# weiyithu/PV-RAFT

Measured on NVIDIA H100. Metric: raft_sample_iters_per_sec, higher is better.
Workload: dtype f32

## Files before the change

pvraft_b200/csrc/corr_lookup.cu:

```cuda
#include <math.h>

#include "fixed_point.cuh"
#include "tma.cuh"

namespace pvraft {

constexpr int kLookupThreads = 640;
constexpr int kAccCells = 128;

__host__ __device__ constexpr size_t lookup_warp_bytes(int K) {
    return (((size_t)(K < 512 ? 512 : K) * 2 + (size_t)K * 4 + 256 + 128 + 2 * kAccCells * 4 + 16) + 127) & ~(size_t)127;
}

struct LookupParams {
    const void* corr_val;
    const void* corr_idx;
    const float4* tab;
    const float* coords;
    float* vox;
    float4* knn_sel;
    int32_t* knn_slot;
    double* moments;
    int8_t* dbg_cube;
    int B, N, K, levels;
    int M;
    int vox_ld;
    float r[4];
    float inv_r[4];
    float thr_c;
    int warps;
    int chunk;
};

template <bool POW2>
__device__ __forceinline__ float div_r(float d, float r, float inv_r) {
    return POW2 ? __fmul_rn(d, inv_r) : __fdiv_rn(d, r);
}

template <bool POW2>
__device__ __forceinline__ unsigned cell_code(float dx, float dy, float dz, float r, float inv_r) {
    const float qx = rintf(div_r<POW2>(dx, r, inv_r));
    const float qy = rintf(div_r<POW2>(dy, r, inv_r));
    const float qz = rintf(div_r<POW2>(dz, r, inv_r));
    const bool ok = fmaxf(fmaxf(fabsf(qx), fabsf(qy)), fabsf(qz)) <= 1.f;
    const int cell = (int)fmaf(qx, 9.f, fmaf(qy, 3.f, qz + 13.f));
    return ok ? (unsigned)cell : 0xFFu;
}

__device__ __forceinline__ void prefetch_row(const void* row, int bytes, int lane) {
    const char* r = reinterpret_cast<const char*>(row);
    if (bytes <= 2048) {
        if (lane * 64 < bytes) asm volatile("prefetch.global.L2 [%0];" ::"l"(r + lane * 64));
    } else {
        for (int o = lane * 64; o < bytes; o += 32 * 64) asm volatile("prefetch.global.L2 [%0];" ::"l"(r + o));
    }
}

template <bool HALF> struct StateT { using val = float; using idx = int32_t; };
template <> struct StateT<true> { using val = uint16_t; using idx = uint16_t; };
__device__ __forceinline__ float load_val(const float* p) { return __ldg(p); }
__device__ __forceinline__ float load_val(const uint16_t* p) { return __uint_as_float((unsigned)__ldg(p) << 16); }

__device__ __forceinline__ unsigned warp_scan_packed(unsigned w, int lane) {
#pragma unroll
    for (int o = 1; o < 32; o <<= 1) {
        const unsigned a = __shfl_up_sync(kFull, w, o);
        if (lane >= o) w += a;
    }
    return w;
}

__device__ __forceinline__ double moments_reduce_scatter(double (&v)[16], int lane) {
#pragma unroll
    for (int d = 16, h = 8; d >= 2; d >>= 1, h >>= 1) {
        const bool up = (lane & d) != 0;
#pragma unroll
        for (int i = 0; i < h; ++i) {
            const double send = up ? v[i] : v[i + h];
            const double keep = up ? v[i + h] : v[i];
            v[i] = keep + __shfl_xor_sync(kFull, send, d);
        }
    }
    return v[0] + __shfl_xor_sync(kFull, v[0], 1);
}

template <int KPL, bool POW2, bool SMEM_TAB, bool HALF, bool DET>
__global__ void __launch_bounds__(kLookupThreads, 1) k_corr_lookup(const LookupParams p) {
    using val_t = typename StateT<HALF>::val;
    using idx_t = typename StateT<HALF>::idx;
    const val_t* g_val = reinterpret_cast<const val_t*>(p.corr_val);
    const idx_t* g_idx = reinterpret_cast<const idx_t*>(p.corr_idx);
    constexpr int VEC = KPL >= 4 ? 4 : KPL;
    constexpr int NJ = KPL / VEC;
    constexpr int K = KPL * 32;
    constexpr unsigned NIB = (1u << VEC) - 1u;
    extern __shared__ __align__(128) unsigned char smem_raw[];
    const size_t tab_bytes = SMEM_TAB ? (((size_t)p.M * 16 + 127) & ~(size_t)127) : 0;
    const float4* s_tab = reinterpret_cast<const float4*>(smem_raw);
    const int w = warp_id();
    int lane;
    asm volatile("mov.u32 %0, %%laneid;" : "=r"(lane));
    unsigned char* wbase = smem_raw + tab_bytes + (size_t)w * lookup_warp_bytes(K);
    int* s_stage = reinterpret_cast<int*>(wbase);
    constexpr int VL = (K < 512 ? 512 : K) * 2;
    unsigned short* s_vlist = reinterpret_cast<unsigned short*>(wbase + K * 4);
    int* s_hist = reinterpret_cast<int*>(wbase + K * 4);
    int* s_slots = reinterpret_cast<int*>(wbase + K * 4 + VL + 256);
    float* s_acc = reinterpret_cast<float*>(wbase + K * 4 + VL + 384);
    int* s_cnt = reinterpret_cast<int*>(wbase + K * 4 + VL + 384 + kAccCells * 4);
    unsigned long long* s_bar = reinterpret_cast<unsigned long long*>(wbase + K * 4 + VL + 384 + 2 * kAccCells * 4);
    pdl_trigger();
    const bool active_warp = w < p.warps;
    __shared__ int s_next;
    __shared__ unsigned long long s_tabbar;
    double* s_rcp = reinterpret_cast<double*>(smem_raw + tab_bytes + (size_t)p.warps * lookup_warp_bytes(K));
    for (int i = threadIdx.x; i <= K; i += blockDim.x) s_rcp[i] = i > 0 ? 1.0 / (double)min(i, p.N) : 1.0;

    if (active_warp && lane == 0) mbar_init(s_bar, 1);
    if (threadIdx.x == 0) mbar_init(&s_tabbar, 1);
    fence_mbarrier_init();
    __syncthreads();

    const bool dyn = p.moments != nullptr && (int)gridDim.x >= p.B;
    const long long total = (long long)p.B * p.N;
    long long pt_begin, pt_end;
    if (dyn) {
        const int b = (int)((long long)blockIdx.x * p.B / gridDim.x);
        pt_begin = (long long)b * p.N;
        pt_end = pt_begin + p.N;
    } else {
        split_range(total, gridDim.x, blockIdx.x, pt_begin, pt_end);
    }
    const int L = p.levels;
    const int nvox = L * 27;
    const unsigned lt_mask = (1u << lane) - 1u;
    unsigned phase = 0, tab_phase = 0;
    bool waited = false;
    const int kChunk = p.chunk;
    const unsigned one = (unsigned)min(p.chunk, 1);

    long long seg = pt_begin;
    while (seg < pt_end) {
        const int b = (int)(seg / p.N);
        long long seg_end = (long long)(b + 1) * p.N;
        if (seg_end > pt_end) seg_end = pt_end;
        const float4* tab_g = p.tab + (size_t)b * p.M;
        int* counter = dyn ? reinterpret_cast<int*>(p.moments + (size_t)b * PVRAFT_MOMENTS + 15) : nullptr;
        if constexpr (DET)
            counter = dyn ? reinterpret_cast<int*>(reinterpret_cast<unsigned long long*>(p.moments) + ((size_t)b * PVRAFT_MOMENTS + 15) * kFxWords) : nullptr;
        auto claim_chunk = [&]() -> long long {
            int c = 0;
            if (lane == 0) c = atomicAdd(counter, kChunk);
            return seg + __shfl_sync(kFull, c, 0);
        };
        __syncthreads();
        if (SMEM_TAB && threadIdx.x == 0) {
            asm volatile("fence.proxy.async.shared::cta;" ::: "memory");
            const unsigned bytes = (unsigned)p.M * 16u;
            mbar_expect_tx(&s_tabbar, bytes);
            for (unsigned off = 0; off < bytes; off += 32768u)
                bulk_g2s(smem_raw + off, reinterpret_cast<const unsigned char*>(tab_g) + off, min(32768u, bytes - off), &s_tabbar);
        }
        if (threadIdx.x == 0) s_next = 2 * p.warps;
        if (!waited) { pdl_wait(); waited = true; }
        long long pt0 = seg + w, nxt0 = seg + w + p.warps;
        int left0 = 0;
        if (dyn && active_warp) { pt0 = claim_chunk(); nxt0 = pt0 + 1; left0 = kChunk - 2; }
        if (active_warp && pt0 < seg_end) {
            if (lane == 0) {
                mbar_expect_tx(s_bar, K * sizeof(idx_t));
                bulk_g2s(s_stage, g_idx + pt0 * K, K * sizeof(idx_t), s_bar);
            }
            prefetch_row(g_val + pt0 * K, K * sizeof(val_t), lane);
        }
        if (SMEM_TAB) { mbar_wait(&s_tabbar, tab_phase); tab_phase ^= 1u; }
        __syncthreads();
        double mom[14];
#pragma unroll
        for (int i = 0; i < 14; ++i) mom[i] = 0.0;
        Fx fmom{0ull, 0ull, 0u};

        if (active_warp) {
            int left = left0, done = 0;
            long long nxt = nxt0;
            for (long long pt = pt0; pt < seg_end; ++done) {
                const float cx = __ldg(p.coords + pt * 3 + 0);
                const float cy = __ldg(p.coords + pt * 3 + 1);
                const float cz = __ldg(p.coords + pt * 3 + 2);
                const val_t* rv = g_val + pt * K;
                const idx_t* ri = g_idx + pt * K;
                if (p.dbg_cube) {
                    for (int i = lane; i < K * L; i += 32) p.dbg_cube[pt * K * L + i] = (int8_t)-1;
                }
                *reinterpret_cast<float4*>(s_acc + lane * 4) = make_float4(0.f, 0.f, 0.f, 0.f);
                *reinterpret_cast<int4*>(s_cnt + lane * 4) = make_int4(0, 0, 0, 0);
                mbar_wait(s_bar, phase);
                phase ^= 1u;

                unsigned dist[KPL];
                unsigned valid_bits = 0;
                const float thr = p.thr_c;
#pragma unroll
                for (int j = 0; j < NJ; ++j) {
                    int ci[VEC];
                    if (VEC == 4 && HALF) {
                        const uint2 c = reinterpret_cast<const uint2*>(s_stage)[j * 32 + lane];
                        ci[0] = (int)(c.x & 0xFFFFu); ci[1 % VEC] = (int)(c.x >> 16); ci[2 % VEC] = (int)(c.y & 0xFFFFu); ci[3 % VEC] = (int)(c.y >> 16);
                    } else if (VEC == 4) {
                        const int4 c = reinterpret_cast<const int4*>(s_stage)[j * 32 + lane];
                        ci[0] = c.x; ci[1 % VEC] = c.y; ci[2 % VEC] = c.z; ci[3 % VEC] = c.w;
                    } else {
#pragma unroll
                        for (int s = 0; s < VEC; ++s) ci[s] = (int)reinterpret_cast<const idx_t*>(s_stage)[j * 32 * VEC + lane * VEC + s];
                    }
#pragma unroll
                    for (int s = 0; s < VEC; ++s) {
                        const float4 q = SMEM_TAB ? s_tab[ci[s]] : __ldg(tab_g + ci[s]);
                        const float dx = __fsub_rn(q.x, cx), dy = __fsub_rn(q.y, cy);
                        const float sx = __fmul_rn(dx, dx), sy = __fmul_rn(dy, dy);
                        const float dz = __fsub_rn(q.z, cz);
                        const float d2 = __fadd_rn(__fadd_rn(sx, sy), __fmul_rn(dz, dz));
                        dist[j * VEC + s] = __float_as_uint(d2);
                        const float amax = fmaxf(fmaxf(fabsf(dx), fabsf(dy)), fabsf(dz));
                        valid_bits |= (amax < thr ? 1u : 0u) << (j * VEC + s);
                    }
                }
                __syncwarp();
                if (nxt < seg_end) {
                    if (lane == 0) {
                        asm volatile("fence.proxy.async.shared::cta;" ::: "memory");
                        mbar_expect_tx(s_bar, K * sizeof(idx_t));
                        bulk_g2s(s_stage, g_idx + nxt * K, K * sizeof(idx_t), s_bar);
                    }
                    prefetch_row(g_val + nxt * K, K * sizeof(val_t), lane);
                }

                if (__any_sync(kFull, valid_bits != 0u)) {
                    int list_n = 0;
                    unsigned w0 = 0, w1 = 0;
#pragma unroll
                    for (int j = 0; j < NJ; ++j) {
                        const unsigned c = __popc((valid_bits >> (j * VEC)) & NIB);
                        if (j < 4) w0 |= c << (8 * j); else w1 |= c << (8 * (j - 4));
                    }
                    const unsigned i0 = warp_scan_packed(w0, lane);
                    const unsigned t0 = __shfl_sync(kFull, i0, 31);
                    unsigned i1 = 0, t1 = 0;
                    if (NJ > 4) { i1 = warp_scan_packed(w1, lane); t1 = __shfl_sync(kFull, i1, 31); }
                    const unsigned e0 = i0 - w0, e1 = i1 - w1;
#pragma unroll
                    for (int j = 0; j < NJ; ++j) {
                        const unsigned ex = j < 4 ? (e0 >> (8 * j)) & 0xFFu : (e1 >> (8 * (j - 4))) & 0xFFu;
                        const unsigned tt = j < 4 ? (t0 >> (8 * j)) & 0xFFu : (t1 >> (8 * (j - 4))) & 0xFFu;
                        unsigned nib = (valid_bits >> (j * VEC)) & NIB;
                        int pos = list_n + (int)ex;
                        while (nib) {
                            const int s = __ffs(nib) - 1;
                            nib &= nib - 1;
                            s_vlist[pos++] = (unsigned short)(j * 32 * VEC + lane * VEC + s);
                        }
                        list_n += (int)tt;
                    }
                    __syncwarp();
                    for (int c0 = 0; c0 < list_n; c0 += 32) {
                        const int n = min(32, list_n - c0);
                        unsigned code = 0xFFFFFFFFu;
                        float val = 0.f;
                        if (lane < n) {
                            const int slot = s_vlist[c0 + lane];
                            const int id = (int)__ldg(ri + slot);
                            val = load_val(rv + slot);
                            const float4 q = SMEM_TAB ? s_tab[id] : __ldg(tab_g + id);
                            const float dx = __fsub_rn(q.x, cx), dy = __fsub_rn(q.y, cy), dz = __fsub_rn(q.z, cz);
#pragma unroll
                            for (int l = 0; l < 4; ++l) {
                                if (l < L) {
                                    const unsigned c = cell_code<POW2>(dx, dy, dz, p.r[l], p.inv_r[l]);
                                    code = (code & ~(0xFFu << (8 * l))) | (c << (8 * l));
                                    if (p.dbg_cube) p.dbg_cube[(pt * K + slot) * L + l] = (int8_t)c;
                                }
                            }
                        }
#pragma unroll
                        for (int l = 0; l < 4; ++l) {
                            if (l < L) {
                                const unsigned c = (code >> (8 * l)) & 0xFFu;
                                const bool act = c != 0xFFu;
                                if (__any_sync(kFull, act)) {
                                    const unsigned m = __match_any_sync(kFull, c);
                                    const unsigned rank = __popc(m & lt_mask), gsize = __popc(m);
                                    const unsigned maxg = __reduce_max_sync(kFull, act ? gsize : 0u);
                                    const int cell = act ? l * 27 + (int)c : 0;
                                    if (act && rank == 0u) s_cnt[cell] += (int)gsize;
                                    for (unsigned r = 0; r < maxg; ++r) {
                                        if (act && rank == r) s_acc[cell] = __fadd_rn(s_acc[cell], val);
                                        __syncwarp();
                                    }
                                }
                            }
                        }
                    }
                }
                __syncwarp();
                {
                    float* vo = p.vox + pt * p.vox_ld;
#pragma unroll
                    for (int i = 0; i < 3; ++i) {
                        const int o = lane + 32 * i;
                        const float v = (float)((double)s_acc[o] * s_rcp[s_cnt[o]]);
                        if (o < p.vox_ld) vo[o] = v;
                    }
                    for (int o = lane + 96; o < p.vox_ld; o += 32) vo[o] = o < nvox ? (float)((double)s_acc[o] * s_rcp[s_cnt[o]]) : 0.f;
                }
                __syncwarp();

                unsigned lmin = dist[0];
#pragma unroll
                for (int e = 1; e < KPL; ++e) lmin = min(lmin, dist[e]);
                unsigned hi = __reduce_max_sync(kFull, lmin);
                unsigned lo;
                int c_lo, c_hi;
                {
                    const unsigned base = hi > 0x01FFFFFFu ? hi - 0x01FFFFFFu : 0u;
                    *reinterpret_cast<int4*>(s_hist + lane * 4) = make_int4(0, 0, 0, 0);
                    __syncwarp();
                    unsigned char* hist_b = reinterpret_cast<unsigned char*>(s_hist);
                    const unsigned dummy = 512u + 4u * (unsigned)lane;
#pragma unroll
                    for (int e = 0; e < KPL; ++e) {
                        const unsigned off = ((max(dist[e], base) - base) >> 16) & 0x1FCu;
                        atomicAdd(reinterpret_cast<unsigned*>(hist_b + (dist[e] <= hi ? off : dummy)), one);
                    }
                    __syncwarp();
                    const int4 h = *reinterpret_cast<const int4*>(s_hist + lane * 4);
                    const int mine = h.x + h.y + h.z + h.w;
                    int incl = mine;
#pragma unroll
                    for (int o = 1; o < 32; o <<= 1) {
                        const int a = __shfl_up_sync(kFull, incl, o);
                        if (lane >= o) incl += a;
                    }
                    const int src = __ffs(__ballot_sync(kFull, incl >= PVRAFT_KNN)) - 1;
                    int c = incl - mine, bq = 0, cl = c, ch = c + h.x;
                    if (ch < PVRAFT_KNN) { cl = ch; ch += h.y; bq = 1; }
                    if (ch < PVRAFT_KNN) { cl = ch; ch += h.z; bq = 2; }
                    if (ch < PVRAFT_KNN) { cl = ch; ch += h.w; bq = 3; }
                    const int B = __shfl_sync(kFull, lane * 4 + bq, src);
                    c_lo = __shfl_sync(kFull, cl, src);
                    c_hi = __shfl_sync(kFull, ch, src);
                    lo = B == 0 ? 0u : base + ((unsigned)B << 18);
                    hi = base + ((unsigned)(B + 1) << 18) - 1u;
                }
                while (c_hi != PVRAFT_KNN && lo < hi) {
                    const unsigned mid = lo + ((hi - lo) >> 1);
                    int c = 0;
#pragma unroll
                    for (int e = 0; e < KPL; ++e) c += dist[e] <= mid ? 1 : 0;
                    c = __reduce_add_sync(kFull, c);
                    if (c >= PVRAFT_KNN) { hi = mid; c_hi = c; } else { lo = mid + 1; c_lo = c; }
                }
                const unsigned T = hi;
                if (c_hi == PVRAFT_KNN) {
                    unsigned m_le = 0;
#pragma unroll
                    for (int e = 0; e < KPL; ++e) m_le |= (dist[e] <= T ? 1u : 0u) << e;
                    int off = __popc(m_le);
                    const int n_le = off;
#pragma unroll
                    for (int o = 1; o < 32; o <<= 1) {
                        const int a = __shfl_up_sync(kFull, off, o);
                        if (lane >= o) off += a;
                    }
                    off -= n_le;
                    while (m_le) {
                        const int e = __ffs(m_le) - 1;
                        m_le &= m_le - 1;
                        s_slots[off++] = (e / VEC) * 32 * VEC + lane * VEC + (e % VEC);
                    }
                } else {
                    unsigned m_lt = 0, m_eq = 0;
#pragma unroll
                    for (int e = 0; e < KPL; ++e) {
                        m_lt |= (dist[e] < T ? 1u : 0u) << e;
                        m_eq |= (dist[e] == T ? 1u : 0u) << e;
                    }
                    const int n_lt = __popc(m_lt), n_eq = __popc(m_eq);
                    int off_lt = n_lt, off_eq = n_eq;
#pragma unroll
                    for (int o = 1; o < 32; o <<= 1) {
                        const int a = __shfl_up_sync(kFull, off_lt, o), c = __shfl_up_sync(kFull, off_eq, o);
                        if (lane >= o) { off_lt += a; off_eq += c; }
                    }
                    const int tot_lt = __shfl_sync(kFull, off_lt, 31);
                    off_lt -= n_lt;
                    off_eq += tot_lt - n_eq;
                    while (m_lt) {
                        const int e = __ffs(m_lt) - 1;
                        m_lt &= m_lt - 1;
                        s_slots[off_lt++] = (e / VEC) * 32 * VEC + lane * VEC + (e % VEC);
                    }
                    while (m_eq) {
                        const int e = __ffs(m_eq) - 1;
                        m_eq &= m_eq - 1;
                        if (off_eq < PVRAFT_KNN) s_slots[off_eq] = (e / VEC) * 32 * VEC + lane * VEC + (e % VEC);
                        ++off_eq;
                    }
                }
                __syncwarp();
                {
                    const int slot = s_slots[lane];
                    const float c = load_val(rv + slot);
                    const int id = (int)__ldg(ri + slot);
                    const float4 q = SMEM_TAB ? s_tab[id] : __ldg(tab_g + id);
                    const float dx = __fsub_rn(q.x, cx), dy = __fsub_rn(q.y, cy), dz = __fsub_rn(q.z, cz);
                    p.knn_sel[pt * 32 + lane] = make_float4(c, dx, dy, dz);
                    if (p.knn_slot) p.knn_slot[pt * 32 + lane] = slot;
                    const double f0 = c, f1 = dx, f2 = dy, f3 = dz;
                    mom[0] += f0; mom[1] += f1; mom[2] += f2; mom[3] += f3;
                    mom[4] += f0 * f0; mom[5] += f0 * f1; mom[6] += f0 * f2; mom[7] += f0 * f3;
                    mom[8] += f1 * f1; mom[9] += f1 * f2; mom[10] += f1 * f3;
                    mom[11] += f2 * f2; mom[12] += f2 * f3; mom[13] += f3 * f3;
                }
                if (DET && p.moments) {
                    double v[16];
#pragma unroll
                    for (int i = 0; i < 14; ++i) { v[i] = mom[i]; mom[i] = 0.0; }
                    v[14] = 1.0;
                    v[15] = 0.0;
                    const double t = moments_reduce_scatter(v, lane);
                    if ((lane & 1) == 0) fx_add(fmom, fx_from(t));
                }
                __syncwarp();
                pt = nxt;
                if (dyn) {
                    if (left > 0) { ++nxt; --left; } else { nxt = claim_chunk(); left = kChunk - 1; }
                } else {
                    int claim = 0;
                    if (lane == 0) claim = atomicAdd(&s_next, 1);
                    nxt = seg + __shfl_sync(kFull, claim, 0);
                }
            }
            if (DET && p.moments) {
                const int which = (lane >> 1) & 15;
                if ((lane & 1) == 0 && which < 15)
                    fx_atomic(reinterpret_cast<unsigned long long*>(p.moments) + ((size_t)b * PVRAFT_MOMENTS + which) * kFxWords, fmom);
            } else if (p.moments) {
                double v[16];
#pragma unroll
                for (int i = 0; i < 14; ++i) v[i] = mom[i];
                v[14] = (double)done;
                v[15] = 0.0;
#pragma unroll
                for (int d = 16, h = 8; d >= 2; d >>= 1, h >>= 1) {
                    const bool up = (lane & d) != 0;
#pragma unroll
                    for (int i = 0; i < h; ++i) {
                        const double send = up ? v[i] : v[i + h];
                        const double keep = up ? v[i + h] : v[i];
                        v[i] = keep + __shfl_xor_sync(kFull, send, d);
                    }
                }
                v[0] += __shfl_xor_sync(kFull, v[0], 1);
                const int which = (lane >> 1) & 15;
                if ((lane & 1) == 0 && which < 15 && v[0] != 0.0) atomicAdd(p.moments + (size_t)b * PVRAFT_MOMENTS + which, v[0]);
            }
        }
        seg = seg_end;
    }
}

__global__ void k_xyz_pad(const float* __restrict__ xyz, long long rows, float4* __restrict__ out) {
    const long long i = (long long)blockIdx.x * blockDim.x + threadIdx.x;
    if (i < rows) out[i] = make_float4(__ldg(xyz + 3 * i), __ldg(xyz + 3 * i + 1), __ldg(xyz + 3 * i + 2), 0.f);
}

template <int KPL>
__global__ void __launch_bounds__(256) k_corr_reorder(const float* __restrict__ val_in, const int32_t* __restrict__ idx_in,
                                                       long long rows, float* __restrict__ val_out, int32_t* __restrict__ idx_out) {
    constexpr int VEC = KPL >= 4 ? 4 : KPL;
    constexpr int K = KPL * 32;
    constexpr int CAP = 4 * KPL;
    __shared__ int s_cur[8][32];
    const int lane = lane_id(), w = warp_id();
    const long long row = (long long)blockIdx.x * 8 + w;
    if (row >= rows) return;
    const unsigned lt_mask = (1u << lane) - 1u;
    float v[KPL];
    int id[KPL];
    int rank[KPL];
    s_cur[w][lane] = 0;
    __syncwarp();
#pragma unroll
    for (int e = 0; e < KPL; ++e) {
        v[e] = __ldg(val_in + row * K + e * 32 + lane);
        id[e] = __ldg(idx_in + row * K + e * 32 + lane);
        const int c = id[e] & 7;
        const unsigned m = __match_any_sync(kFull, c);
        rank[e] = s_cur[w][c] + __popc(m & lt_mask);
        __syncwarp();
        if (lane == __ffs(m) - 1) s_cur[w][c] += __popc(m);
        __syncwarp();
    }
    {
        const int n = lane < 8 ? s_cur[w][lane] : 0;
        const int fr = lane < 8 ? max(0, CAP - n) : 0, ov = lane < 8 ? max(0, n - CAP) : 0;
        int f = fr, o = ov;
#pragma unroll
        for (int d = 1; d < 8; d <<= 1) {
            const int a = __shfl_up_sync(kFull, f, d), c = __shfl_up_sync(kFull, o, d);
            if (lane >= d) { f += a; o += c; }
        }
        if (lane < 8) { s_cur[w][8 + lane] = f - fr; s_cur[w][16 + lane] = o - ov; }
    }
    __syncwarp();
#pragma unroll
    for (int e = 0; e < KPL; ++e) {
        int c = id[e] & 7, k = rank[e];
        if (k >= CAP) {
            const int oi = s_cur[w][16 + c] + (k - CAP);
            int cc = 0;
#pragma unroll
            for (int q = 1; q < 8; ++q) cc = s_cur[w][8 + q] <= oi && s_cur[w][q] < CAP ? q : cc;
            c = cc;
            k = s_cur[w][cc] + (oi - s_cur[w][8 + cc]);
        }
        const int g = k >> 2, ln = c + 8 * (k & 3);
        const int slot = (g / VEC) * 32 * VEC + ln * VEC + (g % VEC);
        val_out[row * K + slot] = v[e];
        idx_out[row * K + slot] = id[e];
    }
}

static bool is_pow2f(float r) {
    int e;
    return r > 0.f && frexpf(r, &e) == 0.5f;
}

static float cube_threshold(float r) {
    volatile float t = 1.5f * r;
    auto q = [&](float x) { volatile float v = x / r; return (float)v; };
    while (q(t) >= 1.5f) t = nextafterf(t, 0.f);
    while (q(t) < 1.5f) t = nextafterf(t, INFINITY);
    return t;
}

static bool lookup_table_in_smem(long long M, int K) {
    const size_t tab = (((size_t)M * 16 + 127) & ~(size_t)127);
    const size_t rcp_bytes = (size_t)(K + 1) * sizeof(double) + 8;
    return tab + 8 * lookup_warp_bytes(K) + rcp_bytes <= (size_t)kSmemBudget;
}

template <int KPL, bool POW2, bool HALF, bool DET>
static int launch_lookup(LookupParams& p, cudaStream_t st) {
    const int K = KPL * 32;
    const size_t per_warp = lookup_warp_bytes(K);
    const size_t tab = (((size_t)p.M * 16 + 127) & ~(size_t)127);
    const size_t rcp_bytes = (size_t)(K + 1) * sizeof(double) + 8;
    const bool smem_tab = lookup_table_in_smem(p.M, K);
    const size_t avail = (size_t)kSmemBudget - (smem_tab ? tab : 0) - rcp_bytes;
    int warps = (int)(avail / per_warp);
    if (warps > kLookupThreads / 32) warps = kLookupThreads / 32;
    if (warps < 1) return fail(PVRAFT_ERR_SMEM, "corr_lookup: K=%d does not fit shared memory", K);
    p.warps = warps;
    p.chunk = 2;
    const size_t rcp = (size_t)(K + 1) * sizeof(double) + 8;
    const size_t smem = (smem_tab ? tab : 0) + warps * per_warp + rcp;
    const long long total = (long long)p.B * p.N;
    int grid = sm_count();
    if ((long long)grid * warps > total) grid = (int)((total + warps - 1) / warps);
    if (grid < 1) grid = 1;
    int rc;
    if (smem_tab) {
        auto k = k_corr_lookup<KPL, POW2, true, HALF, DET>;
        if ((rc = opt_in_smem(k, smem))) return rc;
        launch_pdl(k, grid, kLookupThreads, smem, st, p);
    } else {
        auto k = k_corr_lookup<KPL, POW2, false, HALF, DET>;
        if ((rc = opt_in_smem(k, smem))) return rc;
        launch_pdl(k, grid, kLookupThreads, smem, st, p);
    }
    return check_launch("corr_lookup");
}

}

using namespace pvraft;

extern "C" int pvraft_corr_reorder(const float* val_in, const int32_t* idx_in, int64_t rows, int K, float* val_out,
                                   int32_t* idx_out, void* stream) {
    if (!val_in || !idx_in || !val_out || !idx_out || rows <= 0) return fail(PVRAFT_ERR_BAD_ARG, "corr_reorder: bad argument");
    if (val_in == val_out || idx_in == idx_out) return fail(PVRAFT_ERR_BAD_ARG, "corr_reorder: in-place operation is not supported");
    const unsigned blocks = (unsigned)((rows + 7) / 8);
    cudaStream_t st = (cudaStream_t)stream;
    switch (K) {
        case 32: k_corr_reorder<1><<<blocks, 256, 0, st>>>(val_in, idx_in, rows, val_out, idx_out); break;
        case 64: k_corr_reorder<2><<<blocks, 256, 0, st>>>(val_in, idx_in, rows, val_out, idx_out); break;
        case 128: k_corr_reorder<4><<<blocks, 256, 0, st>>>(val_in, idx_in, rows, val_out, idx_out); break;
        case 256: k_corr_reorder<8><<<blocks, 256, 0, st>>>(val_in, idx_in, rows, val_out, idx_out); break;
        case 512: k_corr_reorder<16><<<blocks, 256, 0, st>>>(val_in, idx_in, rows, val_out, idx_out); break;
        case 1024: k_corr_reorder<32><<<blocks, 256, 0, st>>>(val_in, idx_in, rows, val_out, idx_out); break;
        default: return fail(PVRAFT_ERR_UNSUPPORTED, "corr_reorder: truncate_k=%d (supported: 32,64,128,256,512,1024)", K);
    }
    return check_launch("corr_reorder");
}

extern "C" int pvraft_corr_lookup_table_in_smem(int M, int K) { return M > 0 && K > 0 && lookup_table_in_smem(M, K) ? 1 : 0; }

extern "C" int pvraft_xyz_pad_fwd(const float* xyz, int64_t rows, float* out, void* stream) {
    if (!xyz || !out || rows <= 0) return fail(PVRAFT_ERR_BAD_ARG, "xyz_pad: bad argument");
    k_xyz_pad<<<(unsigned)((rows + 255) / 256), 256, 0, (cudaStream_t)stream>>>(xyz, rows, reinterpret_cast<float4*>(out));
    return check_launch("xyz_pad");
}

template <bool DET>
static int corr_lookup_any(const void* corr_val, const void* corr_idx, bool half, const float* xyz2_pad, const float* coords, int B, int N,
                           int M, int K, int levels, float base_scale, float* vox, int vox_ld, float* knn_sel, int32_t* knn_slot, double* moments,
                           int8_t* dbg_cube, void* ws, void* stream) {
    if (!corr_val || !corr_idx || !xyz2_pad || !coords || !vox || !knn_sel) return fail(PVRAFT_ERR_BAD_ARG, "corr_lookup: null pointer");
    if (B <= 0 || N <= 0 || M <= 0) return fail(PVRAFT_ERR_BAD_ARG, "corr_lookup: B=%d N=%d M=%d", B, N, M);
    if (levels < 1 || levels > 4) return fail(PVRAFT_ERR_UNSUPPORTED, "corr_lookup: levels=%d (1..4 supported)", levels);
    if (!(base_scale > 0.f)) return fail(PVRAFT_ERR_BAD_ARG, "corr_lookup: base_scale must be > 0");
    if ((reinterpret_cast<uintptr_t>(xyz2_pad) & 15u) || (reinterpret_cast<uintptr_t>(corr_idx) & 15u))
        return fail(PVRAFT_ERR_BAD_ARG, "corr_lookup: xyz2_pad and corr_idx must be 16-byte aligned (bulk copies)");
    if (half && M > 65536)
        return fail(PVRAFT_ERR_UNSUPPORTED, "corr_lookup: uint16 candidate ids need M <= 65536 points in the second cloud (M=%d)", M);
    LookupParams p{};
    p.corr_val = corr_val; p.corr_idx = corr_idx; p.tab = reinterpret_cast<const float4*>(xyz2_pad); p.coords = coords;
    p.vox = vox; p.knn_sel = reinterpret_cast<float4*>(knn_sel); p.knn_slot = knn_slot;
    p.moments = DET && moments ? static_cast<double*>(ws) : moments;
    p.dbg_cube = dbg_cube;
    p.B = B; p.N = N; p.M = M; p.K = K; p.levels = levels;
    p.vox_ld = vox_ld > 0 ? vox_ld : levels * 27;
    if (p.vox_ld < levels * 27 || p.vox_ld > levels * 27 + 32) return fail(PVRAFT_ERR_BAD_ARG, "corr_lookup: vox_ld=%d", vox_ld);
    bool pow2 = true;
    for (int l = 0; l < 4; ++l) {
        const float r = (float)((double)base_scale * (double)(1 << l));
        p.r[l] = r;
        p.inv_r[l] = 1.0f / r;
        if (l < levels && !is_pow2f(r)) pow2 = false;
    }
    p.thr_c = cube_threshold(p.r[levels - 1]);
    cudaStream_t st = (cudaStream_t)stream;
    int rc = 0;
#define PVRAFT_LOOKUP_CASE(KPL_)                                                            \
    case KPL_ * 32:                                                                         \
        rc = pow2 ? launch_lookup<KPL_, true, false, DET>(p, st) : launch_lookup<KPL_, false, false, DET>(p, st); \
        break;
#define PVRAFT_LOOKUP_CASE_H(KPL_)                                                          \
    case KPL_ * 32:                                                                         \
        rc = pow2 ? launch_lookup<KPL_, true, true, DET>(p, st) : launch_lookup<KPL_, false, true, DET>(p, st); \
        break;
    if (half) {
        switch (K) {
            PVRAFT_LOOKUP_CASE_H(4)
            PVRAFT_LOOKUP_CASE_H(8)
            PVRAFT_LOOKUP_CASE_H(16)
            PVRAFT_LOOKUP_CASE_H(32)
            default:
                return fail(PVRAFT_ERR_UNSUPPORTED, "corr_lookup (bf16 state): truncate_k=%d (supported: 128,256,512,1024)", K);
        }
    } else {
    switch (K) {
        PVRAFT_LOOKUP_CASE(1)
        PVRAFT_LOOKUP_CASE(2)
        PVRAFT_LOOKUP_CASE(4)
        PVRAFT_LOOKUP_CASE(8)
        PVRAFT_LOOKUP_CASE(16)
        PVRAFT_LOOKUP_CASE(32)
        default:
            return fail(PVRAFT_ERR_UNSUPPORTED, "corr_lookup: truncate_k=%d (supported: 32,64,128,256,512,1024)", K);
    }
    }
#undef PVRAFT_LOOKUP_CASE
#undef PVRAFT_LOOKUP_CASE_H
    if (rc || !DET || !moments) return rc;
    return fx_flush_f64(static_cast<const unsigned long long*>(ws), B, 15, PVRAFT_MOMENTS, PVRAFT_MOMENTS, moments, st);
}

extern "C" int pvraft_corr_lookup_fwd(const float* corr_val, const int32_t* corr_idx, const float* xyz2_pad, const float* coords, int B,
                                      int N, int M, int K, int levels, float base_scale, float* vox, int vox_ld, float* knn_sel,
                                      int32_t* knn_slot, double* moments, int8_t* dbg_cube, void* det_workspace, void* stream) {
    auto f = det_workspace ? corr_lookup_any<true> : corr_lookup_any<false>;
    return f(corr_val, corr_idx, false, xyz2_pad, coords, B, N, M, K, levels, base_scale, vox, vox_ld, knn_sel, knn_slot, moments, dbg_cube,
             det_workspace, stream);
}

extern "C" int pvraft_corr_lookup_bf16_fwd(const uint16_t* corr_val_bf16, const uint16_t* corr_idx_u16, const float* xyz2_pad,
                                           const float* coords, int B, int N, int M, int K, int levels, float base_scale, float* vox,
                                           int vox_ld, float* knn_sel, int32_t* knn_slot, double* moments, int8_t* dbg_cube,
                                           void* det_workspace, void* stream) {
    auto f = det_workspace ? corr_lookup_any<true> : corr_lookup_any<false>;
    return f(corr_val_bf16, corr_idx_u16, true, xyz2_pad, coords, B, N, M, K, levels, base_scale, vox, vox_ld, knn_sel, knn_slot, moments,
             dbg_cube, det_workspace, stream);
}

extern "C" int64_t pvraft_corr_lookup_det_workspace_bytes(int B) { return (int64_t)B * PVRAFT_MOMENTS * kFxWords * 8; }

__global__ void k_state_pack_bf16(const float* __restrict__ val, const int32_t* __restrict__ idx, long long n, uint16_t* __restrict__ val_out,
                                  uint16_t* __restrict__ idx_out) {
    const long long i = (long long)blockIdx.x * blockDim.x + threadIdx.x;
    if (i >= n) return;
    const unsigned u = __float_as_uint(__ldg(val + i));
    const unsigned r = u + 0x7FFFu + ((u >> 16) & 1u);
    val_out[i] = (u & 0x7F800000u) == 0x7F800000u ? (uint16_t)(u >> 16) : (uint16_t)(r >> 16);
    idx_out[i] = (uint16_t)__ldg(idx + i);
}

extern "C" int pvraft_corr_state_pack_bf16(const float* val, const int32_t* idx, int64_t n, uint16_t* val_out, uint16_t* idx_out, void* stream) {
    if (!val || !idx || !val_out || !idx_out || n <= 0) return fail(PVRAFT_ERR_BAD_ARG, "corr_state_pack_bf16: bad argument");
    k_state_pack_bf16<<<(unsigned)((n + 255) / 256), 256, 0, (cudaStream_t)stream>>>(val, idx, n, val_out, idx_out);
    return check_launch("corr_state_pack_bf16");
}
```

Before: 9762.

## Reorder voxel accumulation after KNN selection and prefetch gathered loads early

```diff
diff --git a/pvraft_b200/csrc/corr_lookup.cu b/pvraft_b200/csrc/corr_lookup.cu
--- a/pvraft_b200/csrc/corr_lookup.cu
+++ b/pvraft_b200/csrc/corr_lookup.cu
@@ -104,10 +104,10 @@
     int* s_stage = reinterpret_cast<int*>(wbase);
     constexpr int VL = (K < 512 ? 512 : K) * 2;
     unsigned short* s_vlist = reinterpret_cast<unsigned short*>(wbase + K * 4);
-    int* s_hist = reinterpret_cast<int*>(wbase + K * 4);
     int* s_slots = reinterpret_cast<int*>(wbase + K * 4 + VL + 256);
     float* s_acc = reinterpret_cast<float*>(wbase + K * 4 + VL + 384);
     int* s_cnt = reinterpret_cast<int*>(wbase + K * 4 + VL + 384 + kAccCells * 4);
+    int* s_hist = reinterpret_cast<int*>(s_acc);
     unsigned long long* s_bar = reinterpret_cast<unsigned long long*>(wbase + K * 4 + VL + 384 + 2 * kAccCells * 4);
     pdl_trigger();
     const bool active_warp = w < p.warps;
@@ -192,8 +192,6 @@
                 if (p.dbg_cube) {
                     for (int i = lane; i < K * L; i += 32) p.dbg_cube[pt * K * L + i] = (int8_t)-1;
                 }
-                *reinterpret_cast<float4*>(s_acc + lane * 4) = make_float4(0.f, 0.f, 0.f, 0.f);
-                *reinterpret_cast<int4*>(s_cnt + lane * 4) = make_int4(0, 0, 0, 0);
                 mbar_wait(s_bar, phase);
                 phase ^= 1u;
 
@@ -235,8 +233,9 @@
                     prefetch_row(g_val + nxt * K, K * sizeof(val_t), lane);
                 }
 
+
+                int list_n = 0;
                 if (__any_sync(kFull, valid_bits != 0u)) {
-                    int list_n = 0;
                     unsigned w0 = 0, w1 = 0;
 #pragma unroll
                     for (int j = 0; j < NJ; ++j) {
@@ -262,57 +261,14 @@
                         list_n += (int)tt;
                     }
                     __syncwarp();
-                    for (int c0 = 0; c0 < list_n; c0 += 32) {
-                        const int n = min(32, list_n - c0);
-                        unsigned code = 0xFFFFFFFFu;
-                        float val = 0.f;
-                        if (lane < n) {
-                            const int slot = s_vlist[c0 + lane];
-                            const int id = (int)__ldg(ri + slot);
-                            val = load_val(rv + slot);
-                            const float4 q = SMEM_TAB ? s_tab[id] : __ldg(tab_g + id);
-                            const float dx = __fsub_rn(q.x, cx), dy = __fsub_rn(q.y, cy), dz = __fsub_rn(q.z, cz);
-#pragma unroll
-                            for (int l = 0; l < 4; ++l) {
-                                if (l < L) {
-                                    const unsigned c = cell_code<POW2>(dx, dy, dz, p.r[l], p.inv_r[l]);
-                                    code = (code & ~(0xFFu << (8 * l))) | (c << (8 * l));
-                                    if (p.dbg_cube) p.dbg_cube[(pt * K + slot) * L + l] = (int8_t)c;
-                                }
-                            }
-                        }
-#pragma unroll
-                        for (int l = 0; l < 4; ++l) {
-                            if (l < L) {
-                                const unsigned c = (code >> (8 * l)) & 0xFFu;
-                                const bool act = c != 0xFFu;
-                                if (__any_sync(kFull, act)) {
-                                    const unsigned m = __match_any_sync(kFull, c);
-                                    const unsigned rank = __popc(m & lt_mask), gsize = __popc(m);
-                                    const unsigned maxg = __reduce_max_sync(kFull, act ? gsize : 0u);
-                                    const int cell = act ? l * 27 + (int)c : 0;
-                                    if (act && rank == 0u) s_cnt[cell] += (int)gsize;
-                                    for (unsigned r = 0; r < maxg; ++r) {
-                                        if (act && rank == r) s_acc[cell] = __fadd_rn(s_acc[cell], val);
-                                        __syncwarp();
-                                    }
-                                }
-                            }
-                        }
-                    }
-                }
-                __syncwarp();
-                {
-                    float* vo = p.vox + pt * p.vox_ld;
-#pragma unroll
-                    for (int i = 0; i < 3; ++i) {
-                        const int o = lane + 32 * i;
-                        const float v = (float)((double)s_acc[o] * s_rcp[s_cnt[o]]);
-                        if (o < p.vox_ld) vo[o] = v;
-                    }
-                    for (int o = lane + 96; o < p.vox_ld; o += 32) vo[o] = o < nvox ? (float)((double)s_acc[o] * s_rcp[s_cnt[o]]) : 0.f;
-                }
-                __syncwarp();
+                }
+                int v_id = 0;
+                float v_val = 0.f;
+                if (lane < list_n) {
+                    const int slot = s_vlist[lane];
+                    v_id = (int)__ldg(ri + slot);
+                    v_val = load_val(rv + slot);
+                }
 
                 unsigned lmin = dist[0];
 #pragma unroll
@@ -333,6 +289,8 @@
                     }
                     __syncwarp();
                     const int4 h = *reinterpret_cast<const int4*>(s_hist + lane * 4);
+                    *reinterpret_cast<float4*>(s_acc + lane * 4) = make_float4(0.f, 0.f, 0.f, 0.f);
+                    *reinterpret_cast<int4*>(s_cnt + lane * 4) = make_int4(0, 0, 0, 0);
                     const int mine = h.x + h.y + h.z + h.w;
                     int incl = mine;
 #pragma unroll
@@ -407,15 +365,69 @@
                     }
                 }
                 __syncwarp();
+                const int k_slot = s_slots[lane];
+                const float k_val = load_val(rv + k_slot);
+                const int k_id = (int)__ldg(ri + k_slot);
+
+                for (int c0 = 0; c0 < list_n; c0 += 32) {
+                    const int n = min(32, list_n - c0);
+                    const int id = v_id;
+                    const float val = v_val;
+                    if (c0 + 32 + lane < list_n) {
+                        const int slot = s_vlist[c0 + 32 + lane];
+                        v_id = (int)__ldg(ri + slot);
+                        v_val = load_val(rv + slot);
+                    }
+                    unsigned code = 0xFFFFFFFFu;
+                    if (lane < n) {
+                        const float4 q = SMEM_TAB ? s_tab[id] : __ldg(tab_g + id);
+                        const float dx = __fsub_rn(q.x, cx), dy = __fsub_rn(q.y, cy), dz = __fsub_rn(q.z, cz);
+#pragma unroll
+                        for (int l = 0; l < 4; ++l) {
+                            if (l < L) {
+                                const unsigned c = cell_code<POW2>(dx, dy, dz, p.r[l], p.inv_r[l]);
+                                code = (code & ~(0xFFu << (8 * l))) | (c << (8 * l));
+                                if (p.dbg_cube) p.dbg_cube[(pt * K + s_vlist[c0 + lane]) * L + l] = (int8_t)c;
+                            }
+                        }
+                    }
+#pragma unroll
+                    for (int l = 0; l < 4; ++l) {
+                        if (l < L) {
+                            const unsigned c = (code >> (8 * l)) & 0xFFu;
+                            const bool act = c != 0xFFu;
+                            if (__any_sync(kFull, act)) {
+                                const unsigned m = __match_any_sync(kFull, c);
+                                const unsigned rank = __popc(m & lt_mask), gsize = __popc(m);
+                                const unsigned maxg = __reduce_max_sync(kFull, act ? gsize : 0u);
+                                const int cell = act ? l * 27 + (int)c : 0;
+                                if (act && rank == 0u) s_cnt[cell] += (int)gsize;
+                                for (unsigned r = 0; r < maxg; ++r) {
+                                    if (act && rank == r) s_acc[cell] = __fadd_rn(s_acc[cell], val);
+                                    __syncwarp();
+                                }
+                            }
+                        }
+                    }
+                }
+                __syncwarp();
                 {
-                    const int slot = s_slots[lane];
-                    const float c = load_val(rv + slot);
-                    const int id = (int)__ldg(ri + slot);
-                    const float4 q = SMEM_TAB ? s_tab[id] : __ldg(tab_g + id);
+                    float* vo = p.vox + pt * p.vox_ld;
+#pragma unroll
+                    for (int i = 0; i < 3; ++i) {
+                        const int o = lane + 32 * i;
+                        const float v = (float)((double)s_acc[o] * s_rcp[s_cnt[o]]);
+                        if (o < p.vox_ld) vo[o] = v;
+                    }
+                    for (int o = lane + 96; o < p.vox_ld; o += 32) vo[o] = o < nvox ? (float)((double)s_acc[o] * s_rcp[s_cnt[o]]) : 0.f;
+                }
+
+                {
+                    const float4 q = SMEM_TAB ? s_tab[k_id] : __ldg(tab_g + k_id);
                     const float dx = __fsub_rn(q.x, cx), dy = __fsub_rn(q.y, cy), dz = __fsub_rn(q.z, cz);
-                    p.knn_sel[pt * 32 + lane] = make_float4(c, dx, dy, dz);
-                    if (p.knn_slot) p.knn_slot[pt * 32 + lane] = slot;
-                    const double f0 = c, f1 = dx, f2 = dy, f3 = dz;
+                    p.knn_sel[pt * 32 + lane] = make_float4(k_val, dx, dy, dz);
+                    if (p.knn_slot) p.knn_slot[pt * 32 + lane] = k_slot;
+                    const double f0 = k_val, f1 = dx, f2 = dy, f3 = dz;
                     mom[0] += f0; mom[1] += f1; mom[2] += f2; mom[3] += f3;
                     mom[4] += f0 * f0; mom[5] += f0 * f1; mom[6] += f0 * f2; mom[7] += f0 * f3;
                     mom[8] += f1 * f1; mom[9] += f1 * f2; mom[10] += f1 * f3;
```

Measured after the change: 9812 (median of 6 runs). No clear change (+0.5%).
